# MathThyMod/GP_emu_UQSA

Measured on AMD Instinct MI355X. Metric: log-marginal-likelihood evals/sec at n=16384 d=10 fp64; 1/2/4/8 GPU, higher is better.
Workload: dtype f64

## Files before the change

gp_emu_uqsa_amd/csrc/gpemu.hip:

```cpp
#include <hip/hip_runtime.h>

#include <algorithm>
#include <array>
#include <atomic>
#include <map>
#include <cmath>
#include <cstdio>
#include <cstdlib>
#include <cstring>
#include <limits>
#include <string>
#include <vector>

#include "../../include/gpemu.h"
#include "gpemu_kernels.hpp"
#include "gpemu_gemm_sched.hpp"
#include "gpemu_small.hpp"
#include "gpemu_tiny.hpp"
#include "gpemu_snb.hpp"
#include "gpemu_ozaki.hpp"
#include "gpemu_pivchol.hpp"
#include "gpemu_postgrad.hpp"
#include "gpemu_postmean.hpp"
#include "gpemu_host_alloc.hpp"
// ... 1289 lines not shown
  for (int ti = 0; ti < NT2; ++ti) c->oz_lauum_ops += 2.0 * OZ_T * OZ_T * (ti + 1) * (double)(np2 - OZ_T * ti) * N;
  c->oz_tri.clear();
  for (const auto& prs : F.plan.tri_pairs) {
    if (!oz_tri_level(c, prs)) continue;
    for (const auto& pr : prs) {
      const OzTriPair q = oz_tri_pair_plan(pr[0], pr[1], pr[2], N, all);
      planes = std::max(planes, q.planes_bytes(N));
      resid = std::max(resid, q.resid_bytes(N));
      scratch = std::max(scratch, (size_t)q.Pa * q.Pb);
      nex = std::max(nex, (size_t)(q.Pa + q.Pb));
      c->oz_tri.push_back(q);
    }
  }
  if (const int hs = (&F == &c->tr) ? F.plan.split_h : 0) {
    const OzTriPair* have = nullptr;
    for (const OzTriPair& q : c->oz_tri)
      if (q.t0 == 0 && q.h == hs && q.t1 == F.NB) have = &q;
    const OzTriPair q = have ? *have : oz_tri_pair_plan(0, hs, F.NB, N, all);
    const int nts = q.Pb / OZ_T;
    const std::vector<unsigned> ls = oz_list(nts, nts, true, [&](int, int) { return (double)q.Pa; });
    c->oz_chol_q = q;
    c->oz_chol_loff = (long long)all.size();
    c->oz_chol_llen = (int)ls.size();
    all.insert(all.end(), ls.begin(), ls.end());
    c->oz_chol_ops = 2.0 * OZ_T * OZ_T * (double)q.Pa * N * (nts * (nts + 1) / 2);
    planes = std::max(planes, (size_t)N * q.Pb * q.Pa);
    resid = std::max(resid, (size_t)N * (nts * (size_t)(nts + 1) / 2) * OZ_T * OZ_T);
    nex = std::max(nex, (size_t)q.Pb);
    c->oz_chol_ready = true;
  }
  CHK(dalloc(c, &c->dozp, planes));
  CHK(dalloc(c, &c->dozr, resid));
  CHK(dalloc(c, &c->dozx, nex));
  CHK(dalloc(c, &c->dozt, scratch));
  CHK(dalloc(c, &c->dozl, all.size()));
  HIPCHK(c, hipMemcpy(c->dozl, all.data(), all.size() * sizeof(unsigned), hipMemcpyHostToDevice));
  c->oz_c = oz_consts(N, np2);
  c->oz_np2 = np2;
  c->oz_npad = c->n_pad;
  return GPE_OK;
}

int oz_gemm_crt(gpe_ctx* c, const OzConst& k, const OzGemm& g, const OzCrt& r, int nti, double ops, double flops64,
                hipStream_t st = nullptr) {
  if (!st) st = c->stream;
  if (c->prof) {
    while (c->oev_used + 2 > c->oev.size()) {
      hipEvent_t e;
      HIPCHK(c, hipEventCreate(&e));
      c->oev.push_back(e);
    }
    HIPCHK(c, hipEventRecord(c->oev[c->oev_used], st));
  }
  hipLaunchKernelGGL(k_oz_gemm, dim3(k.nmod * g.list_len), dim3(256), OZ_LDS, st, g, k);
  if (c->prof) {
    HIPCHK(c, hipEventRecord(c->oev[c->oev_used + 1], st));
    c->oev_used += 2;
    c->oz_launches += 1.0;
    c->oz_ops += ops;
    c->oz_flops64 += flops64;
  }
  const int t1 = r.ti0 + nti;
  hipLaunchKernelGGL(k_oz_crt, dim3((g.tri ? t1 * (t1 + 1) / 2 - r.ti0 * (r.ti0 + 1) / 2 : nti * g.ntj) * 16), dim3(256),
                     0, st, r, k);
  HIPCHK(c, hipGetLastError());
  return GPE_OK;
}
int oz_gemm_crt(gpe_ctx* c, const OzGemm& g, const OzCrt& r, int nti, double ops, double flops64,
                hipStream_t st = nullptr) {
  return oz_gemm_crt(c, c->oz_c, g, r, nti, ops, flops64, st);
}

int chol_schur(gpe_ctx* c, Fact& F, hipStream_t st, bool with_aug) {
  const Plan& pl = F.plan;
  const OzTriPair& q = c->oz_chol_q;
  if (!c->oz_chol_ready || q.h != pl.split_h) return fail(c, GPE_ERR_STATE, "internal error: split Cholesky without an int8 plan");
  if (with_aug) CHK(launch_gemm_range(c, pl.launches[pl.aug_mid], st));
  const long long ld = F.n_pad;
  oz_l21_launch(st, c->oz_c, q, F.A + (long long)q.h * TILE, ld, c->dozp, c->dozx);
  HIPCHK(c, hipGetLastError());
  const int nts = q.Pb / OZ_T;
  const long long pA = (long long)q.Pb * q.Pa, rb = (long long)nts * (nts + 1) / 2 * OZ_T * OZ_T;
  OzGemm g;
  g.a = g.b = OzOpnd{c->dozp, pA, q.Pa, 0};
  g.list = c->dozl + c->oz_chol_loff;
  g.list_len = c->oz_chol_llen;
  g.K = q.Pa;
  g.kbeg = 0;
  g.kend = 0;
  g.tri = 1;
  g.ntj = 0;
  g.res = c->dozr;
  g.res_bytes = rb;
  OzCrt r{c->dozr, rb, 1, 0, c->dozx, c->dozx, F.A + (long long)q.h * TILE * (ld + 1), ld, q.Rb, q.Rb, 1, -1.0};
  r.acc = 1;
  CHK(oz_gemm_crt(c, g, r, nts, c->oz_chol_ops, (double)q.Rb * q.Rb * q.Ra, st));
  c->oz_l21_valid = true;
  return GPE_OK;
}

int lauum_ozaki(gpe_ctx* c, Fact& F) {
  CHK(oz_prepare(c, F));
  const int np = (int)F.n_pad, np2 = c->oz_np2, NT2 = np2 / OZ_T;
  const OzConst& k = c->oz_c;
  const long long pb = oz_plane_bytes(np2), rb = (long long)NT2 * (NT2 + 1) / 2 * OZ_T * OZ_T;
  c->oz_l21_valid = false;
  hipLaunchKernelGGL(k_oz_colexp, dim3((np2 + 3) / 4), dim3(256), 0, c->stream, F.B, (long long)F.n_pad, np, np2,
// ... 749 lines not shown
}

static int posterior_oz(gpe_ctx* c, bool f32, const double* Ks, long long mp, double* V) {
  const int np = (int)c->n_pad, np2 = (np + OZ_T - 1) / OZ_T * OZ_T;
  const int mp2 = (int)((mp + OZ_T - 1) / OZ_T * OZ_T);
  const int N = posterior_nmod(np2, f32), nti = np2 / OZ_T, ntj = mp2 / OZ_T;
  const OzConst k = oz_consts(N, np2);
  hipStream_t st = c->stream;
  if (!c->px_valid || c->px_nmod != N) {
    CHK(grow_buf(c, &c->dpxp, &c->pxp_cap, (size_t)N * np2 * np2));
    CHK(grow_buf(c, &c->dpxe, &c->pxe_cap, (size_t)np2));
    HIPCHK(c, hipMemsetAsync(c->dpxe, 0, (size_t)np2 * sizeof(int), st));
    hipLaunchKernelGGL(k_oz_rowexp<true>, dim3(np2 / 64, (np + 255) / 256), dim3(256), 0, st, c->tr.B, (long long)np,
                       np, np2, np, 2, k.beta, c->dpxe);
    hipLaunchKernelGGL(k_oz_il_to_ex, dim3((np2 + 255) / 256), dim3(256), 0, st, c->dpxe, np2, k.beta);
    hipLaunchKernelGGL(k_oz_split_rect<true>, dim3(np2 / 64, np2 / 64), dim3(256), 0, st, c->tr.B, (long long)np, np,
                       np, 2, c->dpxe, c->dpxp, (long long)np2 * np2, (long long)np2, np2, k);
    HIPCHK(c, hipGetLastError());
    c->px_valid = true;
    c->px_nmod = N;
  }
  const long long pB = (long long)mp2 * np2, rb = (long long)nti * ntj * OZ_T * OZ_T;
  if (c->pl_nti != nti || c->pl_ntj != ntj || (size_t)N * pB > c->pkp_cap || (size_t)mp2 > c->pke_cap ||
      (size_t)N * rb > c->pres_cap)
    HIPCHK(c, hipStreamSynchronize(st));
  if (c->pl_nti != nti || c->pl_ntj != ntj) {
    const std::vector<unsigned> l = oz_list(nti, ntj, false, [&](int ti, int) { return (double)(OZ_T * (ti + 1)); });
    c->pl_nti = c->pl_ntj = 0;
    CHK(grow_buf(c, &c->dpl, &c->pl_cap, l.size()));
    HIPCHK(c, hipMemcpy(c->dpl, l.data(), l.size() * sizeof(unsigned), hipMemcpyHostToDevice));
    c->pl_len = (int)l.size();
    c->pl_nti = nti;
    c->pl_ntj = ntj;
  }
  CHK(grow_buf(c, &c->dpkp, &c->pkp_cap, (size_t)N * pB));
  CHK(grow_buf(c, &c->dpke, &c->pke_cap, (size_t)mp2));
  CHK(grow_buf(c, &c->dpres, &c->pres_cap, (size_t)N * rb));
  hipLaunchKernelGGL(k_oz_rowexp<false>, dim3(mp2 / 4), dim3(256), 0, st, Ks, (long long)np, (int)mp, mp2, np, 0, k.beta,
                     c->dpke);
  hipLaunchKernelGGL(k_oz_split_rect<false>, dim3(mp2, (np2 + 2047) / 2048), dim3(256), 0, st, Ks, (long long)np,
                     (int)mp, np, 0, c->dpke, c->dpkp, pB, (long long)np2, np2, k);
  OzGemm g;
  g.a = OzOpnd{c->dpxp, (long long)np2 * np2, np2, 0};
  g.b = OzOpnd{c->dpkp, pB, np2, 0};
  g.list = c->dpl;
  g.list_len = c->pl_len;
  g.K = np2;
  g.kbeg = 0;
  g.kend = 1;
  g.tri = 0;
  g.ntj = ntj;
  g.res = c->dpres;
  g.res_bytes = rb;
  hipLaunchKernelGGL(k_oz_gemm, dim3(N * g.list_len), dim3(256), OZ_LDS, st, g, k);
  OzCrt r{c->dpres, rb, 0, ntj, c->dpxe, c->dpke, V, (long long)np, np, (int)mp, 0, 1.0};
  hipLaunchKernelGGL(k_oz_crt, dim3((unsigned)(nti * ntj * 16)), dim3(256), 0, st, r, k);
  HIPCHK(c, hipGetLastError());
  return GPE_OK;
}

static int ensure_ainv(gpe_ctx* c) {
  if (c->ainv_valid) return GPE_OK;
  CHK(ensure_linv(c));
  CHK(lauum(c, c->tr));
  c->ainv_valid = true;
  return GPE_OK;
}

int gpe_solve(gpe_ctx* c, int32_t ncols, const double* B, double* X) {
  CHK(check_ready(c));
  if (!c->factor_valid) return fail(c, GPE_ERR_STATE, "no resident factor (call gpe_factor)");
  if (ncols <= 0 || !B || !X) return fail(c, GPE_ERR_ARG, "bad solve args");
  CHK(ensure_linv(c));
  const long long np = c->n_pad, n = c->n;
  for (int c0 = 0; c0 < ncols; c0 += SK_PMAX) {
    const int cc = std::min(SK_PMAX, ncols - c0);
    CHK(ensure_pinned(c, (size_t)np * cc + 64));
    std::memset(c->hpin, 0, (size_t)np * cc * sizeof(double));
    for (long long i = 0; i < n; ++i)
      for (int k = 0; k < cc; ++k) c->hpin[i + k * np] = B[i * ncols + c0 + k];
    HIPCHK(c, hipMemcpyAsync(c->dR2, c->hpin, (size_t)np * cc * sizeof(double), hipMemcpyHostToDevice, c->stream));
    CHK(skinny(c, false, c->tr.B, np, c->NB, c->NB, true, c->dR2, np, cc, c->dZ, np));
    CHK(skinny(c, true, c->tr.B, np, c->NB, c->NB, true, c->dZ, np, cc, c->dWa, np));
    HIPCHK(c, hipMemcpyAsync(c->hpin, c->dWa, (size_t)np * cc * sizeof(double), hipMemcpyDeviceToHost, c->stream));
    HIPCHK(c, hipStreamSynchronize(c->stream));
    for (long long i = 0; i < n; ++i)
      for (int k = 0; k < cc; ++k) X[i * ncols + c0 + k] = c->hpin[i + k * np];
  }
  return GPE_OK;
}

int gpe_sense_pairs(gpe_ctx* c, int32_t J, const double* w, const double* u, int32_t p, const double* Z,
                    double* trace_out, double* quad_out) {
  CHK(check_ready(c));
  if (!c->factor_valid) return fail(c, GPE_ERR_STATE, "no resident factor (call gpe_factor)");
  if (J <= 0 || J > 65535 || p <= 0 || !w || !u || !Z || !trace_out || !quad_out)
    return fail(c, GPE_ERR_ARG, "bad sense_pairs args");
  const int d = c->d;
  const int pchunk = std::min(p, 32);
  const bool wide = d > 32;
  const long long np = c->n_pad, n = c->n;
  const int NB = c->NB;
  CHK(ensure_ainv(c));
  const long long ldp = (long long)J * (1 + p * p);
  CHK(grow_buf(c, &c->dSU, &c->su_cap, (size_t)J * np));
  CHK(grow_buf(c, &c->dSZ, &c->sz_cap, (size_t)np * p));
  CHK(grow_buf(c, &c->dSW, &c->sw_cap, (size_t)J * d));
// ... 1569 lines not shown
```

gp_emu_uqsa_amd/csrc/gpemu_dist.hip:

```cpp
#include <hip/hip_runtime.h>
#include <rccl/rccl.h>

#include <algorithm>
#include <cmath>
#include <map>
#include <cstdlib>
#include <cstring>
#include <string>
#include <vector>

#include "../../include/gpemu.h"
#include "../../include/gpemu_dist.h"
#include "gpemu_kernels.hpp"
#include "gpemu_gemm_sched.hpp"
#include "gpemu_small.hpp"
#include "gpemu_ozaki.hpp"

using namespace gpe;

namespace {

struct DistPairArgs {
  const double* xw;
  const double* F;
// ... 729 lines not shown
  for (TriChunk& tc : h->tri) {
    tc.oz.clear();
    const int a = tc.s / 2;
    if (P != 1 || tc.cw != a || (long long)a * TILE < h->oz_tri_min) continue;
    std::vector<unsigned> lists = all;
    std::vector<OzTriPair> prs;
    bool fits = true;
    for (int t0 = 0; t0 + a < NB; t0 += tc.s) {
      const OzTriPair q = oz_tri_pair_plan(t0, t0 + a, std::min(t0 + tc.s, NB), N, lists);
      fits = fits && q.planes_bytes(N) <= (size_t)N * np2 * Kp && q.resid_bytes(N) <= (size_t)N * h->oz_res_bytes &&
             (size_t)q.Pa * q.Pb <= slab_doubles && q.Pa + q.Pb <= np2;
      prs.push_back(q);
    }
    if (!fits) continue;
    all = lists;
    tc.oz = prs;
  }
  DCHK(dalloc(h, &h->ozp, (size_t)N * np2 * Kp, &h->shared_bytes));
  DCHK(dalloc(h, &h->ozr, (size_t)N * h->oz_res_bytes, &h->shared_bytes));
  DCHK(dalloc(h, &h->ozx, (size_t)np2, &h->shared_bytes));
  DCHK(dalloc(h, &h->ozl, all.size(), &h->shared_bytes));
  DCHK_HIP(h, hipMemcpy(h->ozl, all.data(), all.size() * sizeof(unsigned), hipMemcpyHostToDevice));
  return GPE_OK;
}

int oz_split_rank(gpe_dist* h, const Rank& R) {
  const int np2 = h->oz_np2, Kp = h->oz_kp, Kv = R.nlx * TILE;
  const OzConst& k = h->oz_c;
  hipLaunchKernelGGL(k_oz_rowexp<false>, dim3(np2 / 4), dim3(256), 0, h->stream, R.X, R.ld, (int)h->n_pad, np2, Kv,
                     0, k.beta, h->ozx);
  hipLaunchKernelGGL(k_oz_split_rect<false>, dim3(np2, (Kp + 2047) / 2048), dim3(256), 0, h->stream, R.X, R.ld,
                     (int)h->n_pad, Kv, 0, h->ozx, h->ozp, (long long)np2 * Kp, (long long)Kp, Kp, k);
  DCHK_HIP(h, hipGetLastError());
  return GPE_OK;
}

int oz_slab(gpe_dist* h, const Rank& R, const SlabLaunch& sl, size_t si) {
  const int np2 = h->oz_np2, Kp = h->oz_kp;
  const int ti0 = sl.a0 / 2, ti1 = (sl.a1 + 1) / 2;
  const OzConst& k = h->oz_c;
  OzGemm g;
  g.a = g.b = OzOpnd{h->ozp, (long long)np2 * Kp, (long long)Kp, 0};
  g.list = h->ozl + h->oz_lists[si].first;
  g.list_len = h->oz_lists[si].second;
  g.K = Kp;
  g.kbeg = 3;
  g.kdiv = h->P;
  g.kend = 0;
  g.tri = 1;
  g.ntj = 0;
  g.res = h->ozr;
  g.res_bytes = h->oz_res_bytes;
  g.ti0 = ti0;
  hipLaunchKernelGGL(k_oz_gemm, dim3(k.nmod * g.list_len), dim3(256), OZ_LDS, h->stream, g, k);
  const int rows = sl.a1 * TILE;
  OzCrt r{h->ozr, h->oz_res_bytes, 1, 0, h->ozx, h->ozx, R.slab, (long long)h->slab_rows * TILE, rows, rows, 1, 1.0, ti0};
  const long long nt = (long long)ti1 * (ti1 + 1) / 2 - (long long)ti0 * (ti0 + 1) / 2;
  hipLaunchKernelGGL(k_oz_crt, dim3((unsigned)(nt * 16)), dim3(256), 0, h->stream, r, k);
  DCHK_HIP(h, hipGetLastError());
  return GPE_OK;
}

int ensure_grad(gpe_dist* h) {
  if (h->grad_ready) return GPE_OK;
  const int NB = h->NB, P = h->P, Pc = h->q + 1, d = h->d;
  const long long np = h->n_pad;
  long long slab_doubles = (long long)SLAB_DOUBLES;
  const long long whole = (long long)NB * TILE * np;
  if (whole <= 4 * (long long)SLAB_DOUBLES) slab_doubles = std::max(slab_doubles, whole / P);
  if (const char* e = std::getenv("GPEMU_DIST_SLAB_MB")) slab_doubles = std::max(1ll, std::atoll(e)) << 17;
  h->slab_rows = (int)std::max<long long>(1, std::min<long long>(NB, slab_doubles / (TILE * np)));
  const int tri_rows = h->slab_rows;
  const int nlx0 = (NB - 1) / P + 1;
  const double oz_planes = (double)h->oz_nmod * ((np + OZ_T - 1) / OZ_T * OZ_T) * nlx0 * TILE;
  h->oz_now = h->oz_on && np >= h->oz_min_np && (long long)nlx0 * TILE < (1 << 17) &&
              oz_planes <= (double)h->oz_cap_mb * (1 << 20);
  if (h->oz_now && h->slab_rows < NB && (h->slab_rows & 1)) h->slab_rows = std::max(2, h->slab_rows - 1);
  const long long lds = (long long)h->slab_rows * TILE;
  for (Rank& R : h->ranks) {
    R.nlx = R.rank <= NB - 1 ? (NB - 1 - R.rank) / P + 1 : 0;
    DCHK(dalloc(h, &R.X, (size_t)R.ld * NB * TILE, &R.bytes));
    DCHK(dalloc(h, &R.dZ, (size_t)np * Pc, &R.bytes));
    DCHK(dalloc(h, &R.dR2, (size_t)np * Pc, &R.bytes));
    DCHK(dalloc(h, &R.r2loc, (size_t)R.ld * h->NA * TILE, &R.bytes));
    DCHK_HIP(h, hipMemset(R.r2loc, 0, (size_t)R.ld * h->NA * TILE * sizeof(double)));
    DCHK(dalloc(h, &R.wpart, (size_t)np * h->NA * TILE, &R.bytes));
    R.slab_doubles = (long long)std::max(h->slab_rows, tri_rows) * TILE * np;
    DCHK(dalloc(h, &R.slab, (size_t)R.slab_doubles, &R.bytes));
    DCHK(dalloc(h, &R.csum, (size_t)d + 3, &R.bytes));
  }
  DCHK(dalloc(h, &h->dT2, (size_t)Pc * Pc, &h->shared_bytes));
  DCHK(dalloc(h, &h->cpart, (size_t)NB * (NB + 1) / 2 * (d + 3), &h->shared_bytes));

  std::vector<GemmProb> probs;
  std::vector<MoveDesc> moves;
  h->tri.clear();
  const long long cap = (long long)tri_rows * TILE * np, T2 = (long long)TILE * TILE;
  struct Pair { int t0, h, t1; };
  std::vector<std::pair<int, int>> lev;
  long long g1_need = 0, rv_need = 0;
  for (int s = 2; s / 2 < NB; s *= 2) {
    const int a = s / 2;
    long long g1 = 0, s1 = 0, g2 = 0, s2 = 0;
    for (int t0 = 0; t0 + a < NB; t0 += s) {
      const int b = std::min(t0 + s, NB) - (t0 + a);
      g1 += a; s1 += (a + P - 1) / P; g2 += b; s2 += (b + P - 1) / P;
    }
// ... 135 lines not shown
        p.ksplit = ks;
        p.part = h->wsplit + (size_t)wl.tiles * TILE * TILE;
        p.tcnt = h->wcnt + wl.tiles / ks;
      }
      push_prob(wl, probs, p, false);
    }
    h->wa_l[s] = wl;
    for (int a0 = 0; a0 < NB; a0 += h->slab_rows) {
      SlabLaunch sl;
      sl.a0 = a0;
      sl.a1 = std::min(NB, a0 + h->slab_rows);
      sl.gemm = begin_launch(GEMM_AK_BK, probs);
      for (int a = sl.a0; a < sl.a1; ++a) {
        const int ls = lstart_of(a, P, R.rank), K = std::max(0, (R.nlx - ls) * TILE);
        GemmProb p = mkprob(R.X + (long long)ls * TILE + (long long)a * TILE * R.ld, R.ld,
                            R.X + (long long)ls * TILE, R.ld, R.slab + (long long)(a - a0) * TILE, lds,
                            1, a + 1, K, 0, 1.0, 0.0);
        push_prob(sl.gemm, probs, p, false);
      }
      h->slabs[s].push_back(sl);
    }
  }
  for (auto& v : h->slabs)
    for (SlabLaunch& sl : v) list_launch(sl.gemm, probs, gt);
  if ((int)probs.size() > DIST_DESC_MAX) return dfail(h, GPE_ERR_UNSUPPORTED, "distributed gradient schedule too large");
  if (h->oz_now) DCHK(oz_prepare(h));
  DCHK(dalloc(h, &h->gtiles, std::max<size_t>(gt.size(), 1), &h->shared_bytes));
  if (!gt.empty())
    DCHK_HIP(h, hipMemcpy(h->gtiles, gt.data(), gt.size() * sizeof(unsigned), hipMemcpyHostToDevice));
  DCHK(dalloc(h, &h->gprobs, probs.size(), &h->shared_bytes));
  DCHK_HIP(h, hipMemcpy(h->gprobs, probs.data(), probs.size() * sizeof(GemmProb), hipMemcpyHostToDevice));
  h->grad_ready = true;
  return GPE_OK;
}

int move_launch(gpe_dist* h, int first, int count, int tiles) {
  if (count == 0 || tiles == 0) return GPE_OK;
  hipLaunchKernelGGL(k_dist_move, dim3(tiles), dim3(256), 0, h->cs, h->dmoves + first, count);
  DCHK_HIP(h, hipGetLastError());
  return GPE_OK;
}

int trtri_all(gpe_dist* h) {
  h->cs = h->stream;
  for (const TriChunk& tc : h->tri) {
    if (!tc.oz.empty()) {
      Rank& R = h->ranks[0];
      auto tile = [&](double* M, int i, int j) { return M + (long long)i * TILE + (long long)j * TILE * R.ld; };
      const OzConst& k = h->oz_c;
      for (const OzTriPair& q : tc.oz)
        oz_tri_pair_launches(h->stream, k, q, h->ozl, tile(R.A, q.h, q.t0), tile(R.X, q.t0, q.t0), tile(R.X, q.h, q.h),
                             tile(R.X, q.h, q.t0), R.ld, R.slab, h->ozp, h->ozr, h->ozx, false,
                             [&](const OzGemm& g, const OzCrt& r, int nti, double, double) {
                               hipLaunchKernelGGL(k_oz_gemm, dim3(k.nmod * g.list_len), dim3(256), OZ_LDS, h->stream, g, k);
                               hipLaunchKernelGGL(k_oz_crt, dim3((unsigned)(nti * g.ntj * 16)), dim3(256), 0, h->stream,
                                                  r, k);
                             });
      DCHK_HIP(h, hipGetLastError());
      continue;
    }
    if (h->P > 1) {
      DCHK(move_launch(h, tc.pack0, tc.npack, tc.pack_tiles));
      DCHK(coll_allgather(h, &Rank::trecv, tc.seg1));
      DCHK(move_launch(h, tc.unp1, tc.nunp1, tc.unp1_tiles));
    }
    DCHK(launch(h, tc.m, true));
    if (h->P > 1) {
      DCHK(coll_allgather(h, &Rank::trecv, tc.seg2));
      DCHK(move_launch(h, tc.unp2, tc.nunp2, tc.unp2_tiles));
    }
    DCHK(launch(h, tc.x, true));
  }
  return GPE_OK;
}

int kbuild(gpe_dist* h, int kernel, double nu, double s2, double rscale) {
  double coff, cdiag;
  if (kernel == GPE_KERNEL_ALT_NUG) {
    coff = 1.0;
    cdiag = 1.0 + nu * nu;
  } else {
    coff = 1.0 - nu;
    cdiag = 1.0;
  }
  for (Rank& R : h->ranks) {
    if (R.nloc == 0) continue;
    DistPairArgs a;
    a.xw = h->dXw; a.F = h->dF; a.r = (h->has_r && rscale != 0.0) ? h->dr : nullptr; a.out = R.A;
    a.ld = R.ld; a.ldF = h->n_pad; a.d = h->d; a.n_valid = (int)h->n; a.NB = h->NB; a.nranks = h->P;
    a.rank = R.rank; a.nloc = R.nloc; a.Pc = h->q + 1;
    a.s2 = s2; a.coff = coff; a.cdiag = cdiag; a.rscale = rscale;
    const dim3 grid((unsigned)(R.nloc * (h->NB + h->NA)));
    if (h->d <= 4) hipLaunchKernelGGL(k_dist_kbuild<4>, grid, dim3(256), 0, h->stream, a);
    else if (h->d <= 8) hipLaunchKernelGGL(k_dist_kbuild<8>, grid, dim3(256), 0, h->stream, a);
    else if (h->d <= 10) hipLaunchKernelGGL(k_dist_kbuild<10>, grid, dim3(256), 0, h->stream, a);
    else if (h->d <= 16) hipLaunchKernelGGL(k_dist_kbuild<16>, grid, dim3(256), 0, h->stream, a);
    else if (h->d <= 20) hipLaunchKernelGGL(k_dist_kbuild<20>, grid, dim3(256), 0, h->stream, a);
    else if (h->d <= 32) hipLaunchKernelGGL(k_dist_kbuild<32>, grid, dim3(256), 0, h->stream, a);
    else hipLaunchKernelGGL(k_dist_kbuild_wide, grid, dim3(256), 0, h->stream, a);
    DCHK_HIP(h, hipGetLastError());
  }
  return GPE_OK;
}

int step(gpe_dist* h, int k) {
  const int P = h->P, owner = k % P;
  const long long Kp = (long long)(k - h->gstart[k]) * TILE;
// ... 550 lines not shown
```

gp_emu_uqsa_amd/csrc/gpemu_ozaki.hpp:

```cpp
#pragma once
#include <algorithm>
#include <array>
#include <cmath>
#include <cstdlib>
#include <cstring>
#include <utility>
#include <vector>

namespace gpe {

constexpr int OZ_T = 256;
constexpr int OZ_SK = 64;
constexpr int OZ_NBUF = 4;
constexpr int OZ_OPND = OZ_T * OZ_SK;
constexpr int OZ_LDS = OZ_NBUF * 2 * OZ_OPND;
constexpr int OZ_MAXMOD = 16;
constexpr int OZ_MAX_K = (1 << 17) - 128;

struct OzConst {
  int m[OZ_MAXMOD];
  int c16[OZ_MAXMOD];
  float inv[OZ_MAXMOD];
  double rhi[OZ_MAXMOD];
  double rlo[OZ_MAXMOD];
  double Md;
  int nmod;
  int beta;
};

typedef int oz_v4i __attribute__((ext_vector_type(4)));
typedef int oz_v16i __attribute__((ext_vector_type(16)));

constexpr int OZ_EX_NAN = -(1 << 20), OZ_IL_BAD = 1 << 29;
__device__ __forceinline__ double oz_pmax(double a, double b) { return (a > b || a != a) ? a : b; }
__device__ __forceinline__ int oz_ex_of(double mx, int beta) {
  return !(mx <= 1.7976931348623157e308) ? OZ_EX_NAN : (mx > 0.0 ? (beta - 1) - ilogb(mx) : 0);
}

__host__ __device__ __forceinline__ long long oz_panel_off(int cb, int np2) {
  return (long long)OZ_T * ((long long)cb * np2 - (long long)OZ_T * cb * (cb - 1) / 2);
}
__host__ __device__ __forceinline__ long long oz_plane_bytes(int np2) { return oz_panel_off(np2 / OZ_T, np2); }

static __global__ void __launch_bounds__(256) k_oz_colexp(const double* __restrict__ X, long long ldx, int np,
                                                          int np2, int beta, int* __restrict__ ex) {
  const int lane = threadIdx.x & 63, j = blockIdx.x * 4 + (threadIdx.x >> 6);
  if (j >= np2) return;
  double mx = 0.0;
  if (j < np)
    for (int k = j + lane; k < np; k += 64) mx = oz_pmax(mx, fabs(X[k + (long long)j * ldx]));
  for (int off = 32; off > 0; off >>= 1) mx = oz_pmax(mx, __shfl_xor(mx, off, 64));
  if (lane == 0) ex[j] = oz_ex_of(mx, beta);
}

constexpr int OZ_SPLIT_ROWS = 8;
static __global__ void __launch_bounds__(256) k_oz_split(const double* __restrict__ X, long long ldx, int np,
                                                         int np2, const int* __restrict__ ex, int8_t* __restrict__ planes,
                                                         long long plane_bytes, OzConst cst) {
  const int j = blockIdx.x;
  const int cb = j / OZ_T, r0 = cb * OZ_T;
  const int k0 = r0 + OZ_SPLIT_ROWS * ((int)blockIdx.y * 256 + (int)threadIdx.x);
  if (k0 >= np2) return;
  const int e = ex[j];
  double xs[OZ_SPLIT_ROWS];
  if (j < np && k0 + OZ_SPLIT_ROWS <= np && k0 >= j) {
#pragma unroll
    for (int u = 0; u < OZ_SPLIT_ROWS; u += 2) {
      const double2 v = *reinterpret_cast<const double2*>(X + k0 + u + (long long)j * ldx);
      xs[u] = v.x;
      xs[u + 1] = v.y;
    }
  } else {
#pragma unroll
    for (int u = 0; u < OZ_SPLIT_ROWS; ++u) {
      const int k = k0 + u;
      xs[u] = (k >= j && k < np && j < np) ? X[k + (long long)j * ldx] : 0.0;
    }
  }
#pragma unroll
  for (int u = 0; u < OZ_SPLIT_ROWS; ++u) xs[u] = e == OZ_EX_NAN ? 0.0 : rint(ldexp(xs[u], e));
  const long long ld = np2 - r0;
  int8_t* dst = planes + oz_panel_off(cb, np2) + (long long)(j - r0) * ld + (k0 - r0);
  for (int l = 0; l < cst.nmod; ++l) {
    const double m = (double)cst.m[l], im = 1.0 / m;
    unsigned w[2] = {0u, 0u};
#pragma unroll
    for (int u = 0; u < OZ_SPLIT_ROWS; ++u) {
      const double q = rint(xs[u] * im);
      int r = (int)fma(-q, m, xs[u]);
      r = r > 127 ? r - cst.m[l] : (r < -128 ? r + cst.m[l] : r);
      w[u >> 2] |= ((unsigned)r & 0xffu) << (8 * (u & 3));
    }
    *reinterpret_cast<uint2*>(dst + (long long)l * plane_bytes) = make_uint2(w[0], w[1]);
  }
}

__device__ __forceinline__ void oz_glds16(const int8_t* src, int8_t* dst) {
  __builtin_amdgcn_global_load_lds((const __attribute__((address_space(1))) void*)src,
                                   (__attribute__((address_space(3))) void*)dst, 16, 0, 0);
}
template <int N> __device__ __forceinline__ void oz_vmwait() { asm volatile("s_waitcnt vmcnt(%0)" :: "n"(N) : "memory"); }

struct OzOpnd {
  const int8_t* p;
  long long plane_bytes;
  long long ld;
  int np2;
};
__device__ __forceinline__ const int8_t* oz_tile_rows(const OzOpnd& o, int t, int k, long long& ld) {
  if (o.ld == 0) {
    ld = o.np2 - OZ_T * t;
    return o.p + oz_panel_off(t, o.np2) + (k - OZ_T * t);
  }
  ld = o.ld;
  return o.p + (long long)OZ_T * t * o.ld + k;
}

struct OzGemm {
  OzOpnd a, b;
  const unsigned* list;
  int list_len;
  int K, kbeg, kend;
  int tri, ntj;
  int8_t* res;
  long long res_bytes;
  int kdiv = 1;
  int ti0 = 0;
};
__device__ __forceinline__ long long oz_res_tile(int tri, int ntj, int ti, int tj) {
  return tri ? (long long)ti * (ti + 1) / 2 + tj : (long long)ti * ntj + tj;
}

static __global__ void __launch_bounds__(256, 1) k_oz_gemm(OzGemm g, OzConst cst) {
  extern __shared__ __attribute__((aligned(16))) double lds_d[];
  int8_t* lds = reinterpret_cast<int8_t*>(lds_d);
  const int l = (int)blockIdx.x / g.list_len;
  const unsigned ent = g.list[(int)blockIdx.x - l * g.list_len];
  if (ent == 0xffffffffu) return;
  const int ti = (int)(ent >> 16), tj = (int)(ent & 0xffffu);
  const int kb = g.kbeg == 1 ? OZ_T * ti : (g.kbeg == 2 ? OZ_T * tj : (g.kbeg == 3 ? 128 * ((2 * ti) / g.kdiv) : 0));
  const int ke = g.kend == 1 ? min(g.K, OZ_T * (ti + 1)) : g.K;
  const int tid = threadIdx.x, lane = tid & 63;
  const int wave = __builtin_amdgcn_readfirstlane(tid >> 6);
  const int wm = (wave >> 1) * 128, wn = (wave & 1) * 128;
  OzOpnd oa = g.a, ob = g.b;
  oa.p += (long long)l * oa.plane_bytes;
  ob.p += (long long)l * ob.plane_bytes;
  long long lda, ldb;
  const int kp = (lane & 3) ^ ((lane >> 4) & 3);
  const int8_t* sa = oz_tile_rows(oa, ti, kb, lda);
  const int8_t* sb = oz_tile_rows(ob, tj, kb, ldb);
  sa += (long long)(16 * wave + (lane >> 2)) * lda + 16 * kp;
  sb += (long long)(16 * wave + (lane >> 2)) * ldb + 16 * kp;
  auto stage = [&](int s) {
    int8_t* As = lds + (s & (OZ_NBUF - 1)) * 2 * OZ_OPND;
    int8_t* Bs = As + OZ_OPND;
#pragma unroll
    for (int p = 0; p < 4; ++p) {
      const int w = wave + 4 * p;
      oz_glds16(sa + (long long)p * 64 * lda + (long long)s * OZ_SK, As + 16 * w * OZ_SK);
      oz_glds16(sb + (long long)p * 64 * ldb + (long long)s * OZ_SK, Bs + 16 * w * OZ_SK);
    }
  };
  oz_v16i acc[4][4];
#pragma unroll
  for (int i = 0; i < 4; ++i)
#pragma unroll
    for (int j = 0; j < 4; ++j) acc[i][j] = oz_v16i{};
  const int ns = max(0, ke - kb) / OZ_SK;
  const int r32 = lane & 31, h = lane >> 5, sw = (r32 >> 2) & 3;
  auto frags = [&](int s, int ks, oz_v4i (&af)[4], oz_v4i (&bf)[4]) {
    const int8_t* As = lds + (s & (OZ_NBUF - 1)) * 2 * OZ_OPND;
    const int8_t* Bs = As + OZ_OPND;
    const int slot = ((2 * ks + h) ^ sw) * 16;
#pragma unroll
    for (int i = 0; i < 4; ++i) af[i] = *reinterpret_cast<const oz_v4i*>(As + (wm + 32 * i + r32) * OZ_SK + slot);
#pragma unroll
    for (int j = 0; j < 4; ++j) bf[j] = *reinterpret_cast<const oz_v4i*>(Bs + (wn + 32 * j + r32) * OZ_SK + slot);
  };
  auto mfmas = [&](const oz_v4i (&af)[4], const oz_v4i (&bf)[4]) {
#pragma unroll
    for (int i = 0; i < 4; ++i)
#pragma unroll
      for (int j = 0; j < 4; ++j) acc[i][j] = __builtin_amdgcn_mfma_i32_32x32x32_i8(bf[j], af[i], acc[i][j], 0, 0, 0);
  };
  auto wait_stage = [&](int s) {
    const int later = min(ns - 1, s + 2) - s;
    if (later >= 2) oz_vmwait<16>();
    else if (later == 1) oz_vmwait<8>();
    else oz_vmwait<0>();
    asm volatile("s_waitcnt lgkmcnt(0)" ::: "memory");
    __builtin_amdgcn_s_barrier();
  };
  if (ns > 0) {
    for (int s = 0; s < min(ns, 3); ++s) stage(s);
    oz_v4i ca[4], cb[4], na[4], nb[4];
    wait_stage(0);
    if (ns > 3) stage(3);
    frags(0, 0, ca, cb);
    for (int s = 0; s < ns; ++s) {
      mfmas(ca, cb);
      frags(s, 1, na, nb);
#pragma unroll
      for (int u = 0; u < 8; ++u) {
        __builtin_amdgcn_sched_group_barrier(0x008, 1, 0);
        __builtin_amdgcn_sched_group_barrier(0x100, 1, 0);
      }
      __builtin_amdgcn_sched_group_barrier(0x008, 8, 0);
      __builtin_amdgcn_sched_barrier(0);
      if (s + 1 < ns) {
        wait_stage(s + 1);
        if (s + 4 < ns) stage(s + 4);
        frags(s + 1, 0, ca, cb);
      }
      __builtin_amdgcn_sched_barrier(0);
      mfmas(na, nb);
      __builtin_amdgcn_sched_barrier(0);
    }
  }
  const int m = cst.m[l], c16 = cst.c16[l];
  const float inv = cst.inv[l];
  int8_t* out = g.res + (long long)l * g.res_bytes +
                (oz_res_tile(g.tri, g.ntj, ti, tj) - oz_res_tile(g.tri, g.ntj, g.ti0, 0)) * (OZ_T * OZ_T) +
                ((long long)(wave * 16) * 64 + lane) * 16;
#pragma unroll
  for (int i = 0; i < 4; ++i)
#pragma unroll
    for (int j = 0; j < 4; ++j) {
      unsigned w[4] = {0u, 0u, 0u, 0u};
#pragma unroll
      for (int r = 0; r < 16; ++r) {
        const int a = acc[i][j][r];
        int v = a;
        if (m != 256) {
          const int t = __mul24(a >> 16, c16) + (a & 0xffff);
          const int q = (int)rintf((float)t * inv);
          v = t - __mul24(q, m);
        }
        w[r >> 2] |= ((unsigned)v & 0xffu) << (8 * (r & 3));
      }
      *reinterpret_cast<oz_v4i*>(out + (long long)(4 * i + j) * 64 * 16) = oz_v4i{(int)w[0], (int)w[1], (int)w[2], (int)w[3]};
    }
}

struct OzCrt {
  const int8_t* res;
  long long res_bytes;
  int tri, ntj;
  const int* exr;
  const int* exc;
  double* C;
  long long ldc;
  int rows, cols, lower128;
  double alpha;
  int ti0 = 0;
  int acc = 0;
};
static __global__ void __launch_bounds__(256) k_oz_crt(OzCrt g, OzConst cst) {
  const int t = (int)blockIdx.x >> 4;
  const int u = ((int)blockIdx.x & 15) * 256 + (int)threadIdx.x;
  int ti, tj;
  if (g.tri) {
    const int ta = t + g.ti0 * (g.ti0 + 1) / 2;
    ti = g.ti0;
    while ((ti + 1) * (ti + 2) / 2 <= ta) ++ti;
    tj = ta - ti * (ti + 1) / 2;
  } else {
    ti = g.ti0 + t / g.ntj;
    tj = t % g.ntj;
  }
  const int wave = u >> 10, blk = (u >> 6) & 15, lane = u & 63;
  const int i = blk >> 2, j = blk & 3;
  const int gm = OZ_T * ti + (wave >> 1) * 128 + 32 * i + (lane & 31);
  const int gn0 = OZ_T * tj + (wave & 1) * 128 + 32 * j + 4 * (lane >> 5);
  if (gm >= g.rows || gn0 >= g.cols) return;
  double shi[16], slo[16];
#pragma unroll
  for (int r = 0; r < 16; ++r) shi[r] = slo[r] = 0.0;
  const int8_t* src = g.res + (long long)t * (OZ_T * OZ_T) + (long long)u * 16;
  for (int l = 0; l < cst.nmod; ++l) {
    const oz_v4i w = *reinterpret_cast<const oz_v4i*>(src + (long long)l * g.res_bytes);
    const double rh = cst.rhi[l], rl = cst.rlo[l];
#pragma unroll
    for (int r = 0; r < 16; ++r) {
      const double cv = (double)(int)(int8_t)((unsigned)w[r >> 2] >> (8 * (r & 3)));
      shi[r] = fma(cv, rh, shi[r]);
      slo[r] = fma(cv, rl, slo[r]);
    }
  }
  const int em = g.exr[gm];
  const double sc = g.alpha * cst.Md;
#pragma unroll
  for (int r = 0; r < 16; ++r) {
    const int gn = gn0 + (r & 3) + 8 * (r >> 2);
    if (gn >= g.cols || (g.lower128 && (gm >> 7) < (gn >> 7))) continue;
// ... 335 lines not shown
```

Baseline: 17.23.

## Restructure Ozaki int8 GEMM pipeline with interleaved loads and cheaper residue epilogue

Rewrites the k_oz_gemm main loop so each k-step's global-to-LDS loads are split into per-operand halves and interleaved with MFMAs through sched_group_barriers. The loop is specialised into steady-state and tail phases with compile-time wait counts. Load base pointers are made wave-uniform via readfirstlane, with 32-bit per-lane offsets. The residue-reduction epilogue replaces rintf and mask/shift packing with a magic-number float round and byte-permute packing, templated on whether the modulus is 256. This aims to hide memory latency behind MFMAs and cut VALU work, at the cost of more complex scheduling and possible register pressure.

```diff
diff --git a/gp_emu_uqsa_amd/csrc/gpemu.hip b/gp_emu_uqsa_amd/csrc/gpemu.hip
--- a/gp_emu_uqsa_amd/csrc/gpemu.hip
+++ b/gp_emu_uqsa_amd/csrc/gpemu.hip
@@ -1365,7 +1365,7 @@
     }
     HIPCHK(c, hipEventRecord(c->oev[c->oev_used], st));
   }
-  hipLaunchKernelGGL(k_oz_gemm, dim3(k.nmod * g.list_len), dim3(256), OZ_LDS, st, g, k);
+  oz_gemm_launch(st, g, k);
   if (c->prof) {
     HIPCHK(c, hipEventRecord(c->oev[c->oev_used + 1], st));
     c->oev_used += 2;
@@ -2221,7 +2221,7 @@
   g.ntj = ntj;
   g.res = c->dpres;
   g.res_bytes = rb;
-  hipLaunchKernelGGL(k_oz_gemm, dim3(N * g.list_len), dim3(256), OZ_LDS, st, g, k);
+  oz_gemm_launch(st, g, k);
   OzCrt r{c->dpres, rb, 0, ntj, c->dpxe, c->dpke, V, (long long)np, np, (int)mp, 0, 1.0};
   hipLaunchKernelGGL(k_oz_crt, dim3((unsigned)(nti * ntj * 16)), dim3(256), 0, st, r, k);
   HIPCHK(c, hipGetLastError());
diff --git a/gp_emu_uqsa_amd/csrc/gpemu_dist.hip b/gp_emu_uqsa_amd/csrc/gpemu_dist.hip
--- a/gp_emu_uqsa_amd/csrc/gpemu_dist.hip
+++ b/gp_emu_uqsa_amd/csrc/gpemu_dist.hip
@@ -805,7 +805,7 @@
   g.res = h->ozr;
   g.res_bytes = h->oz_res_bytes;
   g.ti0 = ti0;
-  hipLaunchKernelGGL(k_oz_gemm, dim3(k.nmod * g.list_len), dim3(256), OZ_LDS, h->stream, g, k);
+  oz_gemm_launch(h->stream, g, k);
   const int rows = sl.a1 * TILE;
   OzCrt r{h->ozr, h->oz_res_bytes, 1, 0, h->ozx, h->ozx, R.slab, (long long)h->slab_rows * TILE, rows, rows, 1, 1.0, ti0};
   const long long nt = (long long)ti1 * (ti1 + 1) / 2 - (long long)ti0 * (ti0 + 1) / 2;
@@ -1047,7 +1047,7 @@
         oz_tri_pair_launches(h->stream, k, q, h->ozl, tile(R.A, q.h, q.t0), tile(R.X, q.t0, q.t0), tile(R.X, q.h, q.h),
                              tile(R.X, q.h, q.t0), R.ld, R.slab, h->ozp, h->ozr, h->ozx, false,
                              [&](const OzGemm& g, const OzCrt& r, int nti, double, double) {
-                               hipLaunchKernelGGL(k_oz_gemm, dim3(k.nmod * g.list_len), dim3(256), OZ_LDS, h->stream, g, k);
+                               oz_gemm_launch(h->stream, g, k);
                                hipLaunchKernelGGL(k_oz_crt, dim3((unsigned)(nti * g.ntj * 16)), dim3(256), 0, h->stream,
                                                   r, k);
                              });
diff --git a/gp_emu_uqsa_amd/csrc/gpemu_ozaki.hpp b/gp_emu_uqsa_amd/csrc/gpemu_ozaki.hpp
--- a/gp_emu_uqsa_amd/csrc/gpemu_ozaki.hpp
+++ b/gp_emu_uqsa_amd/csrc/gpemu_ozaki.hpp
@@ -4,6 +4,7 @@
 #include <cmath>
 #include <cstdlib>
 #include <cstring>
+#include <type_traits>
 #include <utility>
 #include <vector>
 
@@ -98,6 +99,11 @@
 __device__ __forceinline__ void oz_glds16(const int8_t* src, int8_t* dst) {
   __builtin_amdgcn_global_load_lds((const __attribute__((address_space(1))) void*)src,
                                    (__attribute__((address_space(3))) void*)dst, 16, 0, 0);
+}
+__device__ __forceinline__ const int8_t* oz_uniform(const int8_t* p) {
+  const unsigned long long u = (unsigned long long)p;
+  const unsigned lo = __builtin_amdgcn_readfirstlane((unsigned)u), hi = __builtin_amdgcn_readfirstlane((unsigned)(u >> 32));
+  return (const int8_t*)(((unsigned long long)hi << 32) | lo);
 }
 template <int N> __device__ __forceinline__ void oz_vmwait() { asm volatile("s_waitcnt vmcnt(%0)" :: "n"(N) : "memory"); }
 
@@ -129,6 +135,46 @@
 };
 __device__ __forceinline__ long long oz_res_tile(int tri, int ntj, int ti, int tj) {
   return tri ? (long long)ti * (ti + 1) / 2 + tj : (long long)ti * ntj + tj;
+}
+
+__device__ __forceinline__ void oz_vmwait_stages(int stages) {
+  static_assert(OZ_NBUF <= 5, "one case per stage that can be in flight");
+  if (stages >= 4) oz_vmwait<32>();
+  else if (stages == 3) oz_vmwait<24>();
+  else if (stages == 2) oz_vmwait<16>();
+  else if (stages == 1) oz_vmwait<8>();
+  else oz_vmwait<0>();
+}
+
+template <bool M256>
+__device__ __forceinline__ void oz_store_residues(const oz_v16i (&acc)[4][4], int m, int c16, float inv, int8_t* out) {
+#pragma clang fp contract(off)
+  const int cm = c16 - 65536, nm = -m;
+#pragma unroll
+  for (int i = 0; i < 4; ++i)
+#pragma unroll
+    for (int j = 0; j < 4; ++j) {
+      unsigned v[16];
+#pragma unroll
+      for (int r = 0; r < 16; ++r) {
+        const int a = acc[i][j][r];
+        if constexpr (M256) {
+          v[r] = (unsigned)a;
+        } else {
+          const int t = __mul24(a >> 16, cm) + a;
+          const float qf = (float)t * inv + 12582912.0f;
+          v[r] = (unsigned)(__mul24(__float_as_int(qf), nm) + t);
+        }
+      }
+      oz_v4i w;
+#pragma unroll
+      for (int u = 0; u < 4; ++u) {
+        const unsigned lo = __builtin_amdgcn_perm(v[4 * u + 1], v[4 * u], 0x0c0c0400u);
+        const unsigned hi = __builtin_amdgcn_perm(v[4 * u + 3], v[4 * u + 2], 0x0c0c0400u);
+        w[u] = (int)__builtin_amdgcn_perm(hi, lo, 0x05040100u);
+      }
+      *reinterpret_cast<oz_v4i*>(out + (long long)(4 * i + j) * 64 * 16) = w;
+    }
 }
 
 static __global__ void __launch_bounds__(256, 1) k_oz_gemm(OzGemm g, OzConst cst) {
@@ -148,19 +194,19 @@
   ob.p += (long long)l * ob.plane_bytes;
   long long lda, ldb;
   const int kp = (lane & 3) ^ ((lane >> 4) & 3);
-  const int8_t* sa = oz_tile_rows(oa, ti, kb, lda);
-  const int8_t* sb = oz_tile_rows(ob, tj, kb, ldb);
-  sa += (long long)(16 * wave + (lane >> 2)) * lda + 16 * kp;
-  sb += (long long)(16 * wave + (lane >> 2)) * ldb + 16 * kp;
-  auto stage = [&](int s) {
-    int8_t* As = lds + (s & (OZ_NBUF - 1)) * 2 * OZ_OPND;
-    int8_t* Bs = As + OZ_OPND;
-#pragma unroll
-    for (int p = 0; p < 4; ++p) {
-      const int w = wave + 4 * p;
-      oz_glds16(sa + (long long)p * 64 * lda + (long long)s * OZ_SK, As + 16 * w * OZ_SK);
-      oz_glds16(sb + (long long)p * 64 * ldb + (long long)s * OZ_SK, Bs + 16 * w * OZ_SK);
-    }
+  const int8_t* ua = oz_tile_rows(oa, ti, kb, lda);
+  const int8_t* ub = oz_tile_rows(ob, tj, kb, ldb);
+  unsigned va[4], vb[4];
+#pragma unroll
+  for (int p = 0; p < 4; ++p) {
+    const unsigned row = (unsigned)(16 * wave + (lane >> 2) + 64 * p);
+    va[p] = row * (unsigned)lda + 16u * (unsigned)kp;
+    vb[p] = row * (unsigned)ldb + 16u * (unsigned)kp;
+  }
+  auto load1 = [&](int s, int u) {
+    int8_t* dst = lds + ((unsigned)s % OZ_NBUF) * 2 * OZ_OPND + (u & 1) * OZ_OPND + 16 * (wave + 4 * (u >> 1)) * OZ_SK;
+    const int8_t* src = oz_uniform(((u & 1) ? ub : ua) + (long long)s * OZ_SK);
+    oz_glds16(src + ((u & 1) ? vb[u >> 1] : va[u >> 1]), dst);
   };
   oz_v16i acc[4][4];
 #pragma unroll
@@ -169,14 +215,16 @@
     for (int j = 0; j < 4; ++j) acc[i][j] = oz_v16i{};
   const int ns = max(0, ke - kb) / OZ_SK;
   const int r32 = lane & 31, h = lane >> 5, sw = (r32 >> 2) & 3;
-  auto frags = [&](int s, int ks, oz_v4i (&af)[4], oz_v4i (&bf)[4]) {
-    const int8_t* As = lds + (s & (OZ_NBUF - 1)) * 2 * OZ_OPND;
+  auto frag1 = [&](int s, int ks, int u, oz_v4i (&af)[4], oz_v4i (&bf)[4]) {
+    const int8_t* As = lds + ((unsigned)s % OZ_NBUF) * 2 * OZ_OPND;
     const int8_t* Bs = As + OZ_OPND;
     const int slot = ((2 * ks + h) ^ sw) * 16;
-#pragma unroll
-    for (int i = 0; i < 4; ++i) af[i] = *reinterpret_cast<const oz_v4i*>(As + (wm + 32 * i + r32) * OZ_SK + slot);
-#pragma unroll
-    for (int j = 0; j < 4; ++j) bf[j] = *reinterpret_cast<const oz_v4i*>(Bs + (wn + 32 * j + r32) * OZ_SK + slot);
+    if (u < 4) af[u] = *reinterpret_cast<const oz_v4i*>(As + (wm + 32 * u + r32) * OZ_SK + slot);
+    else bf[u - 4] = *reinterpret_cast<const oz_v4i*>(Bs + (wn + 32 * (u - 4) + r32) * OZ_SK + slot);
+  };
+  auto frags = [&](int s, int ks, oz_v4i (&af)[4], oz_v4i (&bf)[4]) {
+#pragma unroll
+    for (int u = 0; u < 8; ++u) frag1(s, ks, u, af, bf);
   };
   auto mfmas = [&](const oz_v4i (&af)[4], const oz_v4i (&bf)[4]) {
 #pragma unroll
@@ -184,63 +232,78 @@
 #pragma unroll
       for (int j = 0; j < 4; ++j) acc[i][j] = __builtin_amdgcn_mfma_i32_32x32x32_i8(bf[j], af[i], acc[i][j], 0, 0, 0);
   };
-  auto wait_stage = [&](int s) {
-    const int later = min(ns - 1, s + 2) - s;
-    if (later >= 2) oz_vmwait<16>();
-    else if (later == 1) oz_vmwait<8>();
-    else oz_vmwait<0>();
+  if (ns > 0) {
+    oz_v4i ca[4], cb[4], na[4], nb[4];
+    auto kstep = [&](const oz_v4i (&xa)[4], const oz_v4i (&xb)[4], auto READ, int rs, int rks, oz_v4i (&ya)[4],
+                     oz_v4i (&yb)[4], auto LOAD, int ls, int u0) {
+      mfmas(xa, xb);
+      if constexpr (decltype(READ)::value) {
+        frags(rs, rks, ya, yb);
+#pragma unroll
+        for (int u = 0; u < 8; ++u) {
+          __builtin_amdgcn_sched_group_barrier(0x008, 1, 0);
+          __builtin_amdgcn_sched_group_barrier(0x100, 1, 0);
+        }
+      } else {
+        __builtin_amdgcn_sched_group_barrier(0x008, 8, 0);
+      }
+      if constexpr (decltype(LOAD)::value) {
+#pragma unroll
+        for (int u = 0; u < 4; ++u) {
+          load1(ls, u0 + u);
+          __builtin_amdgcn_sched_group_barrier(0x008, 1, 0);
+          __builtin_amdgcn_sched_group_barrier(0x020, 1, 0);
+          __builtin_amdgcn_sched_group_barrier(0x008, 1, 0);
+        }
+      } else {
+        __builtin_amdgcn_sched_group_barrier(0x008, 8, 0);
+      }
+      __builtin_amdgcn_sched_barrier(0);
+    };
+    auto step = [&](int s, auto NEXT, auto LOADA, auto LOADB) {
+      kstep(ca, cb, std::true_type{}, s, 1, na, nb, LOADA, s + OZ_NBUF - 1, 4);
+      if constexpr (decltype(NEXT)::value) {
+        if constexpr (decltype(LOADB)::value) oz_vmwait<8 * (OZ_NBUF - 2)>();
+        else oz_vmwait_stages(ns - s - 2);
+        asm volatile("s_waitcnt lgkmcnt(0)" ::: "memory");
+        __builtin_amdgcn_s_barrier();
+        __builtin_amdgcn_sched_barrier(0);
+      }
+      kstep(na, nb, NEXT, s + 1, 0, ca, cb, LOADB, s + OZ_NBUF, 0);
+    };
+    constexpr std::true_type Y{};
+    constexpr std::false_type N{};
+    if (ns < OZ_NBUF) {
+      for (int s = 0; s < ns; ++s)
+#pragma unroll
+        for (int u = 0; u < 8; ++u) load1(s, u);
+      oz_vmwait_stages(ns - 1);
+    } else {
+#pragma unroll
+      for (int s = 0; s < OZ_NBUF; ++s)
+#pragma unroll
+        for (int u = 0; u < (s == OZ_NBUF - 1 ? 4 : 8); ++u) load1(s, u);
+      oz_vmwait<8 * (OZ_NBUF - 2) + 4>();
+    }
     asm volatile("s_waitcnt lgkmcnt(0)" ::: "memory");
     __builtin_amdgcn_s_barrier();
-  };
-  if (ns > 0) {
-    for (int s = 0; s < min(ns, 3); ++s) stage(s);
-    oz_v4i ca[4], cb[4], na[4], nb[4];
-    wait_stage(0);
-    if (ns > 3) stage(3);
     frags(0, 0, ca, cb);
-    for (int s = 0; s < ns; ++s) {
-      mfmas(ca, cb);
-      frags(s, 1, na, nb);
-#pragma unroll
-      for (int u = 0; u < 8; ++u) {
-        __builtin_amdgcn_sched_group_barrier(0x008, 1, 0);
-        __builtin_amdgcn_sched_group_barrier(0x100, 1, 0);
-      }
-      __builtin_amdgcn_sched_group_barrier(0x008, 8, 0);
-      __builtin_amdgcn_sched_barrier(0);
-      if (s + 1 < ns) {
-        wait_stage(s + 1);
-        if (s + 4 < ns) stage(s + 4);
-        frags(s + 1, 0, ca, cb);
-      }
-      __builtin_amdgcn_sched_barrier(0);
-      mfmas(na, nb);
-      __builtin_amdgcn_sched_barrier(0);
-    }
-  }
-  const int m = cst.m[l], c16 = cst.c16[l];
-  const float inv = cst.inv[l];
+    int s = 0;
+    for (; s + OZ_NBUF < ns; ++s) step(s, Y, Y, Y);
+    if (ns >= OZ_NBUF) step(s++, Y, Y, N);
+    for (; s + 1 < ns; ++s) step(s, Y, N, N);
+    if (s < ns) step(s, N, N, N);
+  }
+  const int m = cst.m[l];
   int8_t* out = g.res + (long long)l * g.res_bytes +
                 (oz_res_tile(g.tri, g.ntj, ti, tj) - oz_res_tile(g.tri, g.ntj, g.ti0, 0)) * (OZ_T * OZ_T) +
                 ((long long)(wave * 16) * 64 + lane) * 16;
-#pragma unroll
-  for (int i = 0; i < 4; ++i)
-#pragma unroll
-    for (int j = 0; j < 4; ++j) {
-      unsigned w[4] = {0u, 0u, 0u, 0u};
-#pragma unroll
-      for (int r = 0; r < 16; ++r) {
-        const int a = acc[i][j][r];
-        int v = a;
-        if (m != 256) {
-          const int t = __mul24(a >> 16, c16) + (a & 0xffff);
-          const int q = (int)rintf((float)t * inv);
-          v = t - __mul24(q, m);
-        }
-        w[r >> 2] |= ((unsigned)v & 0xffu) << (8 * (r & 3));
-      }
-      *reinterpret_cast<oz_v4i*>(out + (long long)(4 * i + j) * 64 * 16) = oz_v4i{(int)w[0], (int)w[1], (int)w[2], (int)w[3]};
-    }
+  if (m == 256) oz_store_residues<true>(acc, m, 0, 0.0f, out);
+  else oz_store_residues<false>(acc, m, cst.c16[l], cst.inv[l], out);
+}
+
+static inline void oz_gemm_launch(hipStream_t st, const OzGemm& g, const OzConst& k) {
+  hipLaunchKernelGGL(k_oz_gemm, dim3((unsigned)(k.nmod * g.list_len)), dim3(256), OZ_LDS, st, g, k);
 }
 
 struct OzCrt {
```

New measurement: 18.43 (median of 6 runs). 1.07x the previous value.
